# jdidion/atropos

Hardware: AMD Instinct MI355X
Metric: reads/s (whole node) 150 bp SE adapter-align (higher is better)
Workload: dtype int32

## Files before the change

atropos_amd/csrc/filter_core.hpp:

```cpp
#ifndef ATR_FILTER_CORE_HPP
#define ATR_FILTER_CORE_HPP

#include "locate_core.hpp"

namespace atr {

constexpr int FILTER_MAX_M = 64;
constexpr int FILTER_CERT_T = 3;
constexpr int FILTER_CERT_TW = 6;
constexpr int FILTER_BINS = 256;

struct FilterParams {
    uint64_t peq[16];
    int rows;
    int and_mode;
    uint32_t tail;
    int32_t thr_row[FILTER_MAX_M + 1];
    uint32_t cert[FILTER_CERT_T + 1];
    uint64_t cert_sub;
    uint64_t rowsel[4];
    uint32_t tailx[3];
    uint64_t cert64[FILTER_CERT_TW + 1];
};

// ... 106 lines not shown
                bool all = true;
                for (int i = 1; i <= m && all; ++i) if (i != x) all = ok(i, i < x ? o : o - 1);
                threat = all;
            }
        if (!threat) cert |= 1ull << (r - 1);
    }
    return cert;
}

inline FilterParams filter_params(const uint64_t *peq64, const uint8_t *codes, int m, int flags, bool and_mode,
                                  const int16_t *thr, int min_overlap, bool planes_path = false) {
    FilterParams fp;
    fp.rows = m; fp.and_mode = and_mode ? 1 : 0; fp.tail = 0u;
    fp.tailx[0] = fp.tailx[1] = fp.tailx[2] = 0u;
    for (int i = 0; i <= FILTER_MAX_M; ++i)
        fp.thr_row[i] = (i >= 1 && i <= m && i >= min_overlap && ((flags & ATR_STOP_WITHIN_SEQ1) || i == m)) ? (int32_t)thr[i] : -1;
    for (int c = 0; c < 16; ++c) fp.peq[c] = peq64[c];
    (void)planes_path;
    if (filter_narrow_applies(m, flags)) {
        fp.rows = FILTER_NARROW_ROWS;
        for (int c = 0; c < 16; ++c) fp.peq[c] = (peq64[c] >> (64 - m)) & 0xFFFFFFFFull;
        for (int t = 0; t < m - FILTER_NARROW_ROWS; ++t) {
            const uint32_t nib = (uint32_t)(codes[FILTER_NARROW_ROWS + t] & 15u) << (4 * (t & 7));
            if (t < 8) fp.tail |= nib; else fp.tailx[(t >> 3) - 1] |= nib;
        }
    }
    filter_overlap_certificates(codes, m, fp.rows, fp.thr_row, and_mode, fp.cert);
    filter_overlap_certificates64(codes, m, planes_path ? fp.rows : 0, fp.thr_row, and_mode, fp.cert64);
    fp.cert_sub = 0ull;
    fp.rowsel[0] = fp.rowsel[1] = fp.rowsel[2] = fp.rowsel[3] = 0ull;
    if (m <= FILTER_MAX_M && (flags & ATR_STOP_WITHIN_SEQ2) && !(flags & ATR_START_WITHIN_SEQ1) && m >= min_overlap && thr[m] >= 1) {
        const int k = (int)thr[m];
        fp.cert_sub = filter_substitution_certificate(codes, m, k, and_mode);
        if (fp.cert_sub)
            for (int i = 0; i < m; ++i) fp.rowsel[codes[i] == 1 ? 0 : codes[i] == 2 ? 1 : codes[i] == 4 ? 2 : 3] |= 1ull << i;
    }
    return fp;
}

constexpr int BAND_W = 16;
#ifndef ATR_BAND_INTERSECT
#define ATR_BAND_INTERSECT 1
#endif
ATR_DEV uint32_t window_word(int j_lo, int j_hi, bool scan, int rows, bool band) {
    return 0x80000000u | (uint32_t)j_lo | ((uint32_t)j_hi << 10) | (scan ? (1u << 20) : 0u) | ((uint32_t)rows << 21) |
           (band ? (1u << 28) : 0u);
}
ATR_DEV bool window_band(uint32_t w) { return ((w >> 28) & 1u) != 0; }
ATR_DEV int window_rows(uint32_t w) { return (int)((w >> 21) & 0x7Fu); }
ATR_DEV int window_lo(uint32_t w) { return (int)(w & 0x3FFu); }
ATR_DEV int window_hi(uint32_t w) { return (int)((w >> 10) & 0x3FFu); }
ATR_DEV bool window_scan(uint32_t w) { return ((w >> 20) & 1u) != 0; }
ATR_DEV bool window_valid(uint32_t w) { return (w >> 31) != 0; }
ATR_DEV uint32_t last_band_word(int dlo, int top, int span, int width, bool rowm) {
    return window_word(dlo, span | (width << 6), true, top, true) | (rowm ? (1u << 29) : 0u);
}
ATR_DEV int last_band_span(uint32_t w) { return window_hi(w) & 63; }
ATR_DEV int last_band_width(uint32_t w) { return window_hi(w) >> 6; }
ATR_DEV bool last_band_rowm(uint32_t w) { return ((w >> 29) & 1u) != 0; }
constexpr int BAND_BINS = 96, ROWS_BIN0 = 192;
ATR_DEV int triangle_rows(int rows, int n, int j, int k) { return rows - (n - j) + k; }
ATR_DEV bool ragged_rows_bins(bool start_within_seq1) { return !start_within_seq1; }
constexpr int TAIL_COLUMNS = 64;

constexpr int LAST_BIN0 = 32;
ATR_DEV int window_bin(uint32_t w, int m, bool by_rows) {
    const int rows = window_rows(w), start = window_lo(w) >> 3;
    if (window_band(w)) {
        if (window_scan(w)) return LAST_BIN0 + 63 - atr_min(rows, 63);
        const int wide = atr_min(7, atr_max(0, (window_hi(w) - window_lo(w) - m) >> 1));
        return (7 - wide) * 4 + atr_min(3, start >> 4);
    }
    if (rows >= m || !by_rows) return 96 + start;
    return ROWS_BIN0 + atr_min(rows, 63);
}

#ifndef ATR_HOST_EMU
__device__ __forceinline__ void fetch_peq8(const uint2 *peq, uint32_t w, uint2 (&e)[8]) {
#pragma unroll
    for (int b = 0; b < 8; ++b) {
        uint32_t off;
        if (b == 0) off = (w << 3) & 0x78u;
        else asm("v_lshrrev_b32 %0, %1, %2\n\tv_and_b32 %0, 0x78, %0" : "=v"(off) : "n"(4 * b - 3), "v"(w));
        e[b] = *(const uint2 *)((const char *)peq + off);
    }
}
#endif

struct FilterState {
    uint32_t pvl, pvh, mvl, mvh;
    int score;
    uint32_t hits;
    uint32_t nz;
    int zfirst;
    int j_first, j_last;
};

ATR_DEV int filter_row_offset(int m, bool wide) { return (wide ? 64 : 32) - m; }
ATR_DEV int filter_row_offset(int m) { return filter_row_offset(m, m > 32); }

ATR_DEV void filter_init(FilterState &F, const Uniform &u, int mf, bool wide) {
    const int off = filter_row_offset(mf, wide);
    const uint32_t low = off >= 32 ? 0u : ~0u << (off & 31);
    if (wide) { F.pvl = u.sr ? 0u : low; F.pvh = u.sr ? 0u : (off > 32 ? ~0u << (off & 31) : ~0u); }
    else { F.pvl = u.sr ? 0u : low; F.pvh = 0u; }
    F.mvl = F.mvh = 0u;
    F.score = (u.sr ? 0 : mf) - (u.k + 1);
    F.hits = F.nz = 0u;
    F.zfirst = 0;
    F.j_first = F.j_last = 0;
}
ATR_DEV void filter_init(FilterState &F, const Uniform &u, int mf) { filter_init(F, u, mf, mf > 32); }

template <bool WIDE>
ATR_DEV void filter_shift_out2(uint32_t &phl, uint32_t &phh, uint32_t &mhl, uint32_t &mhh, int &score, uint32_t &hits,
                               uint32_t &nz, uint32_t kreg) {
#ifdef ATR_HOST_EMU
    hits = (hits << 1) | ((uint32_t)score >> 31);
    nz = (nz << 1) | (uint32_t)(((uint64_t)(uint32_t)score + (uint64_t)kreg) >> 32);
    const uint32_t pout = WIDE ? phh >> 31 : phl >> 31, mout = WIDE ? mhh >> 31 : mhl >> 31;
    if (WIDE) { phh = (phh << 1) | (phl >> 31); mhh = (mhh << 1) | (mhl >> 31); }
    phl <<= 1; mhl <<= 1;
    score += (int)pout - (int)mout;
#else
    uint64_t c0, c2, c3;
    uint32_t t1, t2;
// ... 123 lines not shown
        const int hoff = off > 32 ? off - 32 : 0, hrows = mf - low_rows;
        const uint32_t q = scan(F.pvh >> hoff, F.mvh >> hoff, low_rows + 1, hrows);
        if (q != 0u) largest = low_rows + hrows - atr_ctz(q);
    }
    if (WIDE) {
        const uint64_t rows = (largest >= 64 ? ~0ull : ((1ull << largest) - 1ull)) << off;
        const uint64_t pv = ((uint64_t)F.pvh << 32) | F.pvl, mv = ((uint64_t)F.mvh << 32) | F.mvl;
        cost_of_largest = atr_popc64(pv & rows) - atr_popc64(mv & rows);
    } else {
        const uint32_t rows = (largest >= 32 ? ~0u : ((1u << largest) - 1u)) << off;
        cost_of_largest = atr_popc64((uint64_t)(F.pvl & rows)) - atr_popc64((uint64_t)(F.mvl & rows));
    }
    d_mf = d;
    row_exact = largest;
    if (tail_rule != 1)
        for (int i = mf + 1; i <= u.m; ++i)
            if ((tail_rule == 2 ? d + (i - mf) : d - (i - mf)) <= fp.thr_row[i]) { largest = i; exact = false; }
    return largest;
}

ATR_DEV uint32_t read_dword(const uint32_t *q, int nchunks, int z8);
template <class P, class DW>
ATR_DEV bool filter_tail_cmp(const P &fp, int T, int jp, DW dw) {
    const uint32_t sh = 4u * (uint32_t)(jp & 7);
    bool ok = true;
    uint32_t lo = dw(jp >> 3);
#pragma unroll
    for (int q = 0; q < FILTER_NARROW_TAIL_EXT / 8; ++q) {
        if (8 * q >= T) break;
        const uint32_t hi = dw((jp >> 3) + q + 1);
        const uint32_t w = sh ? ((lo >> sh) | (hi << (32u - sh))) : lo;
        lo = hi;
        const uint32_t tw = q == 0 ? fp.tail : fp.tailx[q >= 1 ? q - 1 : 0];
        const uint32_t x = fp.and_mode ? (w & tw) : (w ^ tw);
        const int left = T - 8 * q;
        const uint32_t ones = left >= 8 ? 0x11111111u : (0x11111111u & ((1u << (4 * left)) - 1u));
        const uint32_t nz = (x | (x >> 1) | (x >> 2) | (x >> 3)) & ones;
        ok = ok && (fp.and_mode ? nz == ones : nz == 0u);
    }
    return ok;
}
template <class P>
ATR_DEV bool filter_tail_matches(const P &fp, int T, const uint32_t *q, int nchunks, int jp) {
    return filter_tail_cmp(fp, T, jp, [&](int z) { return read_dword(q, nchunks, z); });
}

ATR_DEV uint64_t filter_cert64(const FilterParams &fp, int t) { return fp.cert64[t]; }
template <class P> ATR_DEV uint64_t filter_cert64(const P &, int) { return 0ull; }

struct FilterNoDiag { ATR_DEV_MEMBER uint64_t operator()(int) const { return ~0ull; } };

template <bool WIDE, class P, class TM, class DG = FilterNoDiag>
ATR_DEV uint32_t filter_decide_tm(const FilterState &F, const Uniform &u, const P &fp, TM tm, int n, uint32_t rec[4],
                                  int s = 0, bool have_last = true, DG dg = DG(), int pa_dlo = 0, int pa_dhi = -1) {
    const int mf = fp.rows, T = u.m - mf;
    rec[0] = 0xFFFF0000u; rec[1] = 0; rec[2] = 0; rec[3] = 0;
    if (F.zfirst != 0 && u.m >= u.min_overlap) {
        const int j = F.zfirst + T;
        if (T == 0 || (j <= n && tm(j - T))) {
            rec[0] = (uint32_t)u.m << 16;
            rec[1] = (uint32_t)(j - u.m) | ((uint32_t)j << 16);
            rec[2] = (uint32_t)u.m;
            return 0;
        }
    }
    int cost_l = 0, d_mf = 0, row_e = 0;
    bool exact_l = true;
    const int tail_rule = T == 0 ? 0 : (F.j_first == 0 || F.j_last < n - T - u.k) ? 1 : F.j_first == n ? 2 : 0;
    const int row_l = have_last ? filter_last_column<WIDE>(F, u, fp, cost_l, exact_l, tail_rule, d_mf, row_e) : 0;
    const bool lastcol = row_l != 0;
    const bool rowm = F.j_first != 0 && u.m >= u.min_overlap && !(tail_rule == 2 && d_mf + T > u.k);
    if (!lastcol && !rowm) return 0;
    if (!rowm && !u.sr && exact_l && cost_l == 0) {
        rec[0] = (uint32_t)row_l << 16;
        rec[1] = (uint32_t)(n - row_l) | ((uint32_t)n << 16);
        rec[2] = (uint32_t)row_l;
        return 0;
    }
    if (!WIDE && !rowm && !u.sr && exact_l && u.indel == 1 && cost_l >= 1 && cost_l <= FILTER_CERT_T && row_l > cost_l) {
        const int i = row_l - cost_l, off = filter_row_offset(mf, false);
        const uint32_t seg = ((1u << cost_l) - 1u) << (off + i);
        if ((F.pvl & seg) == seg && ((fp.cert[cost_l] >> i) & 1u) != 0u && n - i >= s) {
            rec[0] = (uint32_t)i << 16;
            rec[1] = (uint32_t)(n - i) | ((uint32_t)n << 16);
            rec[2] = (uint32_t)i;
            return 0;
        }
    }
    if (WIDE && !rowm && !u.sr && exact_l && u.indel == 1 && cost_l >= 1 && cost_l <= FILTER_CERT_TW && row_l > cost_l) {
        const int i = row_l - cost_l, off = filter_row_offset(mf, true);
        const uint64_t seg = ((1ull << cost_l) - 1ull) << (off + i), pv = ((uint64_t)F.pvh << 32) | F.pvl;
        if ((pv & seg) == seg && ((filter_cert64(fp, cost_l) >> i) & 1ull) != 0ull && n - i >= s) {
            rec[0] = (uint32_t)i << 16;
            rec[1] = (uint32_t)(n - i) | ((uint32_t)n << 16);
            rec[2] = (uint32_t)i;
            return 0;
        }
    }
    if (!rowm && !u.sr && exact_l && u.indel == 1) {
        const int kk = atr_min(u.k, (int)fp.thr_row[row_l]), dlo = n - row_l - kk;
        if (dlo >= s && cost_l + 2 * kk <= BAND_W - 1) return last_band_word(dlo, row_l, atr_min(cost_l, row_l - 1), cost_l + 2 * kk, false);
    }
    if (rowm && lastcol && !u.sr && u.indel == 1 && row_e != 0) {
        const int top = exact_l ? row_l : u.m, r0 = atr_max(1, row_e - cost_l);
        const int dlo = atr_min(F.j_first - mf - u.k, n - top - u.k), dhi = atr_max(F.j_last - mf + u.k, n - r0 + u.k);
        if (dlo >= s && dhi - dlo <= BAND_W - 1) return last_band_word(dlo, top, top - r0, dhi - dlo, true);
    }
    int j_lo = 0x7fffffff;
    if (rowm) j_lo = F.j_first - mf - u.k;
    if (lastcol) j_lo = atr_min(j_lo, n - row_l - ((u.indel == 1 && exact_l) ? cost_l : u.k));
    j_lo = atr_max(s, j_lo);
    bool band = rowm && !lastcol && (F.j_first - mf - u.k >= s) &&
                (F.j_last - F.j_first + 2 * u.k <= BAND_W - 1);
    int band_hi = F.j_last + T;
    const bool pa = rowm && !lastcol && !u.sr && pa_dhi >= pa_dlo && pa_dlo > s;
    if (!band && pa && pa_dhi - pa_dlo <= BAND_W - 1) {
        band = true;
        j_lo = pa_dlo;
        band_hi = pa_dhi + u.m - u.k;
    } else if (band && !u.sr && u.indel == 1 && fp.cert_sub != 0ull && ((F.j_first + F.j_last) & 1) == 0 &&
        F.j_last - F.j_first <= 2 * u.k) {
        const int xc = (F.j_first + F.j_last) >> 1, d = xc - mf, j = d + u.m;
        if (d >= s && j <= n) {
            const uint64_t mm = dg(d);
            if (mm != 0ull && (mm & (mm - 1ull)) == 0ull && (mm & fp.cert_sub) != 0ull) {
                rec[0] = (uint32_t)u.m << 16;
                rec[1] = (uint32_t)d | ((uint32_t)j << 16);
                rec[2] = (uint32_t)(u.m - 1) | (1u << 16);
                return 0;
            }
        }
    }
    if (ATR_BAND_INTERSECT && band && pa) {
        const int lo = atr_max(pa_dlo, F.j_first - mf - u.k), hi = atr_min(pa_dhi + u.m - u.k, F.j_last + T);
        if (hi - (u.m - u.k) >= lo) { j_lo = lo; band_hi = hi; }
    }
    const int j_hi = lastcol ? n : band ? band_hi : atr_min(n, F.j_last + (T ? T + u.k : 0));
    return window_word(j_lo, j_hi, lastcol, rowm ? u.m : row_l, band);
}

template <bool WIDE, class P>
ATR_DEV uint32_t filter_decide(const FilterState &F, const Uniform &u, const P &fp, const uint32_t *q,
                               int nchunks, int n, uint32_t rec[4], int s = 0) {
    const int T = u.m - fp.rows;
    return filter_decide_tm<WIDE>(F, u, fp, [&](int jp) { return filter_tail_matches(fp, T, q, nchunks, jp); }, n, rec, s);
}

struct BandParams {
    uint32_t rrep[FILTER_MAX_M];
    int and_mode, noindel;
};

constexpr int BAND_STREAM = (FILTER_MAX_M + BAND_W + 7) / 8 + 1;

ATR_DEV uint32_t read_dword(const uint32_t *q, int nchunks, int z8) {
    if (z8 < 0 || z8 >= nchunks * 4) return 0u;
    return q[(size_t)(z8 >> 2) * 256 + (z8 & 3)];
}

ATR_DEV int band_stream_dwords(int m) { return atr_min(BAND_STREAM, 3 + (m >> 3)); }
ATR_DEV void band_stage(const uint32_t *q, int nchunks, int dlo, uint32_t *ns, int nss, int ndw = BAND_STREAM) {
    const int z0 = dlo >> 3;
    const uint32_t sh = 4u * (uint32_t)(dlo & 7);
    uint32_t raw[BAND_STREAM + 1];
#pragma unroll
    for (int k = 0; k <= BAND_STREAM; ++k) raw[k] = k <= ndw ? read_dword(q, nchunks, z0 + k) : 0u;
#pragma unroll
    for (int k = 0; k < BAND_STREAM; ++k)
        if (k < ndw) ns[(size_t)k * nss] = sh ? ((raw[k] >> sh) | (raw[k + 1] << (32u - sh))) : raw[k];
}

ATR_DEV uint32_t nibble_any(uint32_t v) {
    const uint32_t t = v | (v << 1);
    return t | (t << 2);
}

template <bool AND_MODE, int ND, bool PREFIX = false, class RR>
ATR_DEV void band_rows(const Uniform &u, RR rrep_of, const uint32_t *ns, int nss, uint32_t (&band)[BAND_W]) {
    const uint32_t inf = ((uint32_t)INIT_COST_CAP << CSH) | ORG_BIAS;
    uint32_t qw0 = ns[0], qw1 = ns[(size_t)nss];
    uint32_t feed = ns[(size_t)2 * nss];
    for (int i = 1; i <= u.m; ++i) {
        const uint32_t rrep = rrep_of(i);
        uint32_t m0 = nibble_any(AND_MODE ? (qw0 & rrep) : (qw0 ^ rrep));
        uint32_t m1 = ND > 8 ? nibble_any(AND_MODE ? (qw1 & rrep) : (qw1 ^ rrep)) : 0u;
        if (AND_MODE) { m0 = ~m0; m1 = ~m1; }
        uint32_t left = inf;
        if (PREFIX && i <= u.k) {
            const uint32_t col0 = ORG_BIAS | ((uint32_t)atr_min(i * u.indel, INIT_COST_CAP) << CSH);
#pragma unroll
// ... 215 lines not shown
```

atropos_amd/csrc/locate_core.hpp:

```cpp
#ifndef ATR_LOCATE_CORE_HPP
#define ATR_LOCATE_CORE_HPP

#include <stdint.h>
#include "atropos_hip.h"

#ifdef ATR_HOST_EMU
#define ATR_DEV static inline
#ifndef ATR_DEV_MEMBER
#define ATR_DEV_MEMBER inline
#endif
static inline int atr_min(int a, int b) { return a < b ? a : b; }
static inline int atr_max(int a, int b) { return a > b ? a : b; }
static inline uint32_t atr_minu(uint32_t a, uint32_t b) { return a < b ? a : b; }
static inline uint32_t atr_mad24(uint32_t a, uint32_t b, uint32_t c) { return a * b + c; }
static inline uint32_t atr_bfe1(uint32_t w, int i) { return (w >> i) & 1u; }
static inline int atr_clz(uint32_t w) { return __builtin_clz(w); }
static inline int atr_ctz(uint32_t w) { return __builtin_ctz(w); }
static inline int atr_popc64(uint64_t w) { return __builtin_popcountll(w); }
#else
#define ATR_DEV __device__ __forceinline__
#ifndef ATR_DEV_MEMBER
#define ATR_DEV_MEMBER __device__ __forceinline__
#endif
#define atr_min min
// ... 174 lines not shown
    return u;
}

template <int MT, bool NOINDEL, bool XREP>
ATR_DEV void lane_init(LaneState<MT> &L, const Uniform &u, int n, const uint32_t *s_init, const int16_t *thr) {
    L.n = n;
    L.max_n = u.sq ? n : atr_min(n, u.m + u.k);
    L.min_n = XREP ? 0 : atr_max(0, n - u.m - u.k);
    L.scan = (L.max_n == n);
    if (XREP) {
#pragma unroll
        for (int i = 0; i <= MT; ++i) L.col[i] = s_init[i];
    } else {
#pragma unroll
        for (int i = 0; i <= MT; ++i) L.col[i] = init_word(i - u.p0, L.min_n, u.sr, u.sq, u.indel);
    }
    L.best.key = COST_FIELD_MAX - (u.m + n);
    L.best.word = (uint32_t)(u.m + n) << CSH;
    L.best.ref_stop = u.m; L.best.query_stop = n; L.best.matches = 0;
    if (L.scan && n == 0)
        scan_last_column<MT, XREP>(L.best, L.col, u.p0, u.first_p, n, u.min_overlap, thr, NOINDEL ? 0 : u.indel, u.klimit);
}

ATR_DEV uint32_t window_init_word(int i, int j_lo, int indel) {
    const int cost = i < 0 ? INIT_COST_CAP : atr_min(i * indel, INIT_COST_CAP);
    return ((uint32_t)cost << CSH) | (uint32_t)(j_lo + (int)ORG_BIAS);
}

template <int MT, bool NOINDEL>
ATR_DEV void lane_init_window(LaneState<MT> &L, const Uniform &u, int n, int j_start, int j_hi, bool scan,
                              const uint32_t *s_init, const int16_t *thr) {
    L.n = n; L.min_n = j_start; L.max_n = j_hi; L.scan = scan;
    if (j_start == 0) {
#pragma unroll
        for (int i = 0; i <= MT; ++i) L.col[i] = s_init[i];
    } else {
#pragma unroll
        for (int i = 0; i <= MT; ++i) L.col[i] = window_init_word(i - u.p0, j_start, u.indel);
    }
    L.best.key = COST_FIELD_MAX - (u.m + n);
    L.best.word = (uint32_t)(u.m + n) << CSH;
    L.best.ref_stop = u.m; L.best.query_stop = n; L.best.matches = 0;
    if (scan && j_hi <= j_start)
        scan_last_column<MT, true>(L.best, L.col, u.p0, u.first_p, n, u.min_overlap, thr, NOINDEL ? 0 : u.indel, u.klimit);
}

template <int MT>
ATR_DEV void lane_restart_window(LaneState<MT> &L, const Uniform &u, int j_start) {
#pragma unroll
    for (int i = 0; i <= MT; ++i) L.col[i] = window_init_word(i - u.p0, j_start, u.indel);
    L.best.key = COST_FIELD_MAX - (u.m + L.n);
    L.best.word = (uint32_t)(u.m + L.n) << CSH;
    L.best.ref_stop = u.m; L.best.query_stop = L.n; L.best.matches = 0;
}

template <int MT, bool NOINDEL, bool XREP, bool WIN = false>
ATR_DEV void lane_step(LaneState<MT> &L, const Uniform &u, int j, const uint32_t (&nm)[(MT + 31) / 32],
                       const int16_t *thr, int plimit = MT, int obase = 0) {
    const int indel = NOINDEL ? 0 : u.indel;
    const uint32_t row0 = u.sq ? (ORG_BIAS + (uint32_t)(j - obase))
                               : (ORG_BIAS | ((uint32_t)atr_min(j * u.indel, INIT_COST_CAP) << CSH));
    const uint32_t wm = WIN ? column_step_limited<MT, NOINDEL, XREP>(L.col, nm, u.p0, row0, u.insw, u.delw, plimit)
                            : column_step<MT, NOINDEL, XREP>(L.col, nm, u.p0, row0, u.insw, u.delw);
    if (WIN) {
        if (plimit == MT && wm < u.klimit && j <= L.max_n)
            consider<XREP>(L.best, wm, u.m, j, u.min_overlap, thr, indel);
    } else if (XREP) {
        if (wm < u.klimit && j <= L.max_n) consider<XREP>(L.best, wm, u.m, j, u.min_overlap, thr, indel, obase);
    } else if (j == L.min_n && L.max_n > L.min_n) {
        int mn = L.min_n;
#ifndef ATR_HOST_EMU
        asm volatile("" : "+v"(mn));
#endif
#pragma unroll
        for (int i = 0; i <= MT; ++i) L.col[i] = init_word(i - u.p0, mn, u.sr, u.sq, u.indel) - (uint32_t)obase;
    }
    if (L.scan && j == L.max_n && L.max_n > L.min_n)
        scan_last_column<MT, XREP>(L.best, L.col, u.p0, u.first_p, L.n, u.min_overlap, thr, indel, u.klimit, WIN ? plimit : MT, obase);
}

constexpr int LONG_BASE_STEP = 256, LONG_MAX_SPAN = 384;
ATR_DEV int long_base(int j) { return j > 2 * LONG_BASE_STEP ? (((j - 1) / LONG_BASE_STEP) - 1) * LONG_BASE_STEP : 0; }
template <int MT>
ATR_DEV void lane_rebase(LaneState<MT> &L) {
#pragma unroll
    for (int i = 0; i <= MT; ++i) {
        const uint32_t w = L.col[i];
        L.col[i] = (w & ORG_MASK) >= (uint32_t)LONG_BASE_STEP ? w - (uint32_t)LONG_BASE_STEP : (w & ~ORG_MASK);
    }
}

template <int MT>
ATR_DEV void lane_result(const LaneState<MT> &L, const Uniform &u, uint32_t rec[4], int obase = 0) {
    const int cost = (int)(L.best.word >> CSH);
    int refstart = 0, querystart = 0, refstop = -1, querystop = 0, matches = 0, errors = 0;
    if (L.best.key != COST_FIELD_MAX - (u.m + L.n) && cost != u.m + L.n) {
        const int origin = (int)(L.best.word & ORG_MASK) - (int)ORG_BIAS + obase;
        if (origin >= 0) querystart = origin; else refstart = -origin;
        refstop = L.best.ref_stop; querystop = L.best.query_stop;
        matches = L.best.matches; errors = cost;
    }
    rec[0] = (uint32_t)(refstart & 0xFFFF) | ((uint32_t)(refstop & 0xFFFF) << 16);
    rec[1] = (uint32_t)(querystart & 0xFFFF) | ((uint32_t)(querystop & 0xFFFF) << 16);
    rec[2] = (uint32_t)(matches & 0xFFFF) | ((uint32_t)(errors & 0xFFFF) << 16);
    rec[3] = 0;
}
// ... 45 lines not shown
```

atropos_amd/csrc/locate_fast.hpp:

```cpp
#ifndef ATR_LOCATE_FAST_HPP
#define ATR_LOCATE_FAST_HPP

#include <algorithm>
#include "locate_kernel.hpp"
#include "filter_core.hpp"
#include "linked_core.hpp"
#include "piece_core.hpp"
#include "fast_work.hpp"

namespace atr {
inline const FilterParams &aligner_filter_params(const atr_aligner *a) {
    struct Slot { unsigned long long uid = 0; FilterParams fp; };
    static thread_local Slot slots[4];
    static thread_local unsigned turn = 0;
    if (a->uid != 0)
        for (Slot &s : slots) if (s.uid == a->uid) return s.fp;
    Slot &s = slots[turn++ & 3u];
    s.fp = filter_params(a->peq, a->codes, a->p.m, a->flags, a->wildcard_ref || a->wildcard_query, a->p.thr, a->p.min_overlap);
    s.uid = a->uid;
    return s.fp;
}
inline const FilterParams &aligner_piece_filter_params(const atr_aligner *a) {
    struct Slot { unsigned long long uid = 0; FilterParams fp; };
    static thread_local Slot slots[4];
// ... 257 lines not shown
    __syncthreads();
    const int lane = threadIdx.x & 63;
    const long long tile = (long long)blockIdx.x * 4 + __builtin_amdgcn_readfirstlane((int)(threadIdx.x >> 6));
    if (tile * 64 >= nreads) return;
    const long long r = tile * 64 + lane;
    const bool live = r < nreads;
    const int n = live ? (lens ? lens[r] : max_len) : 0;
    const uint32_t *q = (const uint32_t *)(packed + (size_t)tile * nchunks * 64 + lane);
    uint32_t *ns = &s_stream[__builtin_amdgcn_readfirstlane((int)(threadIdx.x >> 6))][0][lane];
    band_stage(q, nchunks, -u.k, ns, 64, band_stream_dwords(u.m));
    uint32_t rec[4];
    band_locate_prefix<AND_MODE>(u, bp.rrep, bp.noindel != 0, ns, 64, n, s_thr, rec);
    if (live) out[r] = make_uint4(rec[0], rec[1], rec[2], rec[3]);
}
#endif

template <bool LINKED>
__device__ __forceinline__ const LocateParams &window_params(const LocateParams &p_arg, const LinkedArgs &la, int ad) {
    if constexpr (LINKED) return la.multi_p[ad];
    else return p_arg;
}

template <int MT, bool NOINDEL, bool LINKED, bool PLANES = false>
__global__ __launch_bounds__(256) void window_kernel(const LocateParams p_arg, const uint4 *__restrict__ packed,
                                                     const int32_t *__restrict__ lens, long long nreads,
                                                     int nchunks, int max_len, uint4 *__restrict__ out, FastWork wk,
                                                     const LinkedArgs la) {
    __shared__ int16_t s_thr[ATR_MAX_REF_LEN + 2];
    __shared__ uint32_t s_init[ATR_MAX_REF_LEN + 1];
    __shared__ __attribute__((aligned(16))) uint32_t s_nm[16][4];
    __shared__ uint32_t s_spread_flat[PLANES ? 1024 : 1];
    uint32_t (*s_spread)[256] = (uint32_t (*)[256])s_spread_flat;
    const int ad = LINKED ? la.a0 + (int)blockIdx.y : 0;
    const LocateParams &p = window_params<LINKED>(p_arg, la, ad);
    const Uniform u = make_uniform(p, MT);
    if (threadIdx.x < 64) s_nm[threadIdx.x >> 2][threadIdx.x & 3] = p.nmask[threadIdx.x >> 2][threadIdx.x & 3];
    for (int i = threadIdx.x; i <= MT + 1; i += 256) {
        if (i <= u.m + 1) s_thr[i] = p.thr[i];
        if (i <= MT) s_init[i] = init_word(i - u.p0, 0, u.sr, u.sq, u.indel);
    }
    if constexpr (PLANES) piece_spread_fill(s_spread);
    __syncthreads();
    const int bin0 = LINKED ? ad * FILTER_BINS : 0;
    const long long first = (long long)wk.binbase[bin0 + BAND_BINS], total = (long long)wk.binbase[bin0 + FILTER_BINS];
    const int lane = threadIdx.x & 63;
    const int lpw = dp_lanes_per_wave(total - first, (long long)gridDim.x * 4, wk.lpw);
    const long long nwaves = (total - first + lpw - 1) / lpw;
    for (long long wv = (long long)blockIdx.x * 4 + __builtin_amdgcn_readfirstlane((int)(threadIdx.x >> 6)); wv < nwaves;
         wv += (long long)gridDim.x * 4) {
        const long long slot = first + wv * lpw + lane;
        const bool live = lane < lpw && slot < total;
        const uint2 task = live ? wk.order[slot] : make_uint2(0u, 0u);
        const long long r = (long long)task.x;
        const uint32_t ww = task.y;
        const int n = live ? (lens ? lens[r] : max_len) : 0;
        const int j_lo = window_lo(ww), j_hi = live ? window_hi(ww) : 0;
        const bool has_window = live && j_hi > j_lo;
        const int jlo = wave_min_i32(live ? j_lo : 0x7fffffff);
        const int jhi = wave_max_i32(has_window ? j_hi : 0);
        const int rows_w = wave_max_i32(live ? window_rows(ww) : 0);
        const int plimit = u.p0 + rows_w;
        const bool head = !(u.sr && jlo == 0);
        const bool tri = __builtin_amdgcn_readfirstlane((int)(first + wv * lpw >= (long long)wk.binbase[bin0 + ROWS_BIN0])) != 0 &&
                         head && lens == nullptr;
        const int s_lane = (LINKED && live) ? (int)(la.front[r].y >> 16) : 0;
        const int s_top = LINKED ? wave_max_i32(s_lane) : 0;

        LaneState<MT> L;
        const uint4 *tp = packed + ((size_t)(r >> 6) * nchunks) * 64 + (r & 63);

        const bool rows_wave = __builtin_amdgcn_readfirstlane((int)(first + wv * lpw >= (long long)wk.binbase[bin0 + ROWS_BIN0])) != 0;
        if (!LINKED && lens != nullptr && rows_wave && !u.sr) {
            const int shift = live ? max_len - n : 0;
            const int v0 = wave_min_i32(live ? j_lo + shift : 0x7fffffff);
            if (max_len - v0 <= TAIL_COLUMNS && v0 < max_len) {
                const int s_top_t = wave_max_i32(shift);
                lane_init_window<MT, NOINDEL>(L, u, max_len, v0, live ? max_len : 0, live && window_scan(ww), s_init, s_thr);
                uint32_t tb[TAIL_COLUMNS / 8];
                {
                    const int dlo = n - TAIL_COLUMNS;
                    const int z0 = dlo >> 3;
                    const uint32_t sh = 4u * (uint32_t)(dlo & 7);
                    uint32_t raw[TAIL_COLUMNS / 8 + 1];
#pragma unroll
                    for (int t = 0; t <= TAIL_COLUMNS / 8; ++t) {
                        if constexpr (PLANES) raw[t] = live ? read_dword_planes((const uint32_t *)tp, nchunks, z0 + t, s_spread) : 0u;
                        else raw[t] = live ? read_dword((const uint32_t *)tp, nchunks, z0 + t) : 0u;
                    }
#pragma unroll
                    for (int t = 0; t < TAIL_COLUMNS / 8; ++t) tb[t] = sh ? ((raw[t] >> sh) | (raw[t + 1] << (32u - sh))) : raw[t];
                }
                int j = max_len - TAIL_COLUMNS;
#pragma unroll 1
                for (int d = 0; d < TAIL_COLUMNS / 8; ++d) {
                    uint32_t w = tb[0];
#pragma unroll
                    for (int t = 0; t + 1 < TAIL_COLUMNS / 8; ++t) tb[t] = tb[t + 1];
#pragma unroll 1
                    for (int b = 0; b < 8; ++b) {
                        ++j;
                        const uint32_t q = w & 15u;
                        w >>= 4;
                        if (j <= v0) continue;
                        uint32_t nm[(MT + 31) / 32];
                        load_mask(nm, s_nm, q);
                        int pl = min(plimit, u.p0 + (j - v0) + u.k);
                        pl = min(pl, u.p0 + triangle_rows(rows_w, max_len, j, u.k));
                        lane_step<MT, NOINDEL, true, true>(L, u, j, nm, s_thr, pl);
// ... 87 lines not shown
```

atropos_amd/csrc/piece_filter.hpp:

```cpp
#ifndef ATR_PIECE_FILTER_HPP
#define ATR_PIECE_FILTER_HPP

#include "fast_work.hpp"
#include "pack_fast.hpp"

namespace atr {

#ifndef ATR_PIECE_PREFETCH_EARLY
#define ATR_PIECE_PREFETCH_EARLY 1
#endif
#ifndef ATR_PIECE_STASH
#define ATR_PIECE_STASH 1
#endif
#ifndef ATR_PIECE_WAVES
#if defined(ATR_SPEC) && defined(ATR_SPEC_ASCII)
#define ATR_PIECE_WAVES(NW) 2
#elif defined(ATR_SPEC)
#define ATR_PIECE_WAVES(NW) ((NW) <= 6 ? 4 : 3)
#else
#define ATR_PIECE_WAVES(NW) ((NW) <= 6 ? 4 : (NW) <= 8 ? 3 : 2)
#endif
#endif

constexpr int PIECE_QF = 2;
template <bool B> struct PieceBool { static constexpr bool value = B; };

__device__ __forceinline__ int lane_rank(uint64_t mask) {
    return (int)__builtin_amdgcn_mbcnt_hi((uint32_t)(mask >> 32), __builtin_amdgcn_mbcnt_lo((uint32_t)mask, 0u));
}

__device__ __forceinline__ void piece_emit(bool active, long long r, uint32_t ww, const uint32_t (&rec)[4], int m, uint4 *out,
                                           uint2 *list, uint4 *ldata, const uint32_t *nibs, int j0, uint32_t *s_lcur, uint32_t *s_hist,
                                           int nd = 8) {
    const bool open = active && window_valid(ww);
    if (active && !open) out[r] = make_uint4(rec[0], rec[1], rec[2], rec[3]);
    const uint64_t om = __ballot(open);
    if (om != 0ull) {
        uint32_t base = 0u;
        if ((threadIdx.x & 63) == 0) base = atomicAdd(s_lcur, (uint32_t)__popcll(om));
        base = __builtin_amdgcn_readfirstlane(base);
        const int lane = threadIdx.x & 63;
        const int off = window_lo(ww) - j0;
        const bool dense = nibs != nullptr && off >= 0 && off < 64 && band_stream_dwords(m) <= 8;
        if (open) {
            const uint32_t slot = base + (uint32_t)lane_rank(om);
            list[slot] = make_uint2((uint32_t)r, dense ? ww : (ww | PIECE_NODENSE));
            atomicAdd(&s_hist[window_bin(ww, m, true)], 1u);
            if (dense) {
                const int z = off >> 3;
                const uint32_t sh = 4u * (uint32_t)(off & 7);
                uint32_t raw[9], d[8];
#pragma unroll
                for (int k = 0; k < 9; ++k) raw[k] = z + k < nd ? nibs[(z + k) * 64 + lane] : 0u;
#pragma unroll
                for (int k = 0; k < 8; ++k) d[k] = sh ? ((raw[k] >> sh) | (raw[k + 1] << (32u - sh))) : raw[k];
                ldata[2 * (size_t)slot] = make_uint4(d[0], d[1], d[2], d[3]);
                ldata[2 * (size_t)slot + 1] = make_uint4(d[4], d[5], d[6], d[7]);
            }
        }
    }
}

template <int NW, bool RAGGED, int WW = 2>
__device__ __forceinline__ void piece_filter_body(const LocateParams &p, const FilterParams &fp_arg, const PieceParams &pp_arg,
                                                  const uint4 *__restrict__ planes, const int32_t *__restrict__ lens,
                                                  long long nreads, int max_len, uint4 *__restrict__ out, FastWork wk,
                                                  const uint8_t *__restrict__ ascii = nullptr, const uint8_t *tab = nullptr) {
#ifdef ATR_SPEC
    if (!RAGGED) max_len = spec::N;
#endif
#ifdef ATR_SPEC_ASCII
    static_assert(NW <= 8, "the fused ASCII entry keeps pass B's window in the LDS stash");
    constexpr int STRIDE = ATR_SPEC_STRIDE;
    constexpr int NPC = (15 + 64 * STRIDE + 1023) / 1024;
    constexpr int STAGE_BYTES = (64 * STRIDE + PACK_STAGE_SLACK + 15) & ~15;
    __shared__ __attribute__((aligned(16))) uint8_t s_stage[4][STAGE_BYTES];
// ... 92 lines not shown
            nb[d] = 0u;
            if (d >= dw0 - 1) nb[d] = piece_nibbles(s_spread, wp[0][d >> 2], wp[1][d >> 2], wp[2][d >> 2], wp[3][d >> 2], d & 3);
            nibs[d * 64 + lane] = nb[d];
        }
        const auto sweep_decide = [&](auto wc) __attribute__((always_inline)) {
        constexpr bool WD = decltype(wc)::value;
        FilterState F;
        filter_init(F, u, mf, WD);
        int vstart = 0;
        if (u.sr) {
            const bool zero0 = j_e - W <= 0;
            Uniform uf = u;
            uf.sr = false;
            FilterState G;
            filter_init(G, uf, mf, WD);
            if (!zero0) { F.pvl = G.pvl; F.pvh = G.pvh; F.score = G.score; }
            vstart = zero0 ? PW - j_e : 0;
        }
        uint2 ea[8], eb[8];
#pragma unroll
        for (int d = 0; d < ND; ++d) {
            if (d < dw0) continue;
            uint2 (&e)[8] = (d & 1) ? eb : ea;
            if (d == dw0) fetch_peq8(s_peq, nb[d], e);
            if (d + 1 < ND) fetch_peq8(s_peq, nb[d + 1], (d & 1) ? ea : eb);
            if (u.sr) {
#pragma unroll
                for (int b = 0; b < 8; ++b) if (8 * d + b < vstart) { e[b].x = ~0u; e[b].y = ~0u; }
            }
#pragma unroll
            for (int b = 0; b < 8; ++b) filter_step<WD>(F, e[b].x, e[b].y, kreg);
            if ((d & 3) == 3 && d + 1 < ND) filter_fold(F, j_e - PW + 8 * (d + 1), mf, kreg);
        }
        filter_fold(F, j_e, mf, kreg);
        uint32_t rec[4];
        const auto tm = [&](int jp) {
            const int rp = max(0, jp - (j_e - PW));
            return filter_tail_cmp(fp, T, rp, [&](int z) { return z < ND ? nibs[z * 64 + lane] : 0u; });
        };
        const auto dg = [&](int d) -> uint64_t {
            if constexpr (WW != 2 || WD) return ~0ull;
            const int o = d - (j_e - PW);
            if (o < 0 || o + u.m > PW) return ~0ull;
            uint64_t eq = 0ull;
#pragma unroll
            for (int c = 0; c < 4; ++c) {
                uint32_t lo = wp[c][0], hi = wp[c][1];
#pragma unroll
                for (int q = 0; q < 4; ++q) if (q != c && !fp.and_mode) { lo &= ~wp[q][0]; hi &= ~wp[q][1]; }
                eq |= ((((uint64_t)hi << 32) | lo) >> o) & fp.rowsel[c];
            }
            return ~eq & (u.m >= 64 ? ~0ull : (1ull << u.m) - 1ull);
        };
        const uint32_t ww = filter_decide_tm<WD>(F, u, fp, tm, nr, rec, 0, j_e == nr, dg, j_e - need, j_e < nr ? j_e - u.m : -0x10000);
        piece_emit(act, r, ww, rec, u.m, out, list, ldata, nibs, j_e - PW, &s_lcur, s_hist, ND);
        };
        if (mf > 32) {
            if constexpr (WIDE_OK) sweep_decide(PieceBool<true>{});
        } else {
            sweep_decide(PieceBool<false>{});
        }
    };

    int qn = 0;

#ifdef ATR_SPEC_ASCII
    uint4 ax[NPC];
    const auto ascii_edge = [&](long long tile) {
        const uint8_t *src = ascii + tile * 64 * STRIDE;
        const uint8_t *al = src - ((uintptr_t)src & 15);
        const long long need = (long long)((uintptr_t)src & 15) + (nreads - tile * 64 < 64 ? nreads - tile * 64 : 64) * STRIDE;
        return al < ascii || al + ((need + 15) & ~15ll) > buf_end;
    };
    const auto ascii_request = [&](long long tile) {
        if (ascii_edge(tile)) return;
        const uint8_t *src = ascii + tile * 64 * STRIDE;
        const uint8_t *al = src - ((uintptr_t)src & 15);
        const long long need = (long long)((uintptr_t)src & 15) + (nreads - tile * 64 < 64 ? nreads - tile * 64 : 64) * STRIDE;
#pragma unroll
        for (int u = 0; u < NPC; ++u) {
            const long long o = (long long)u * 1024 + (long long)lane * 16;
            ax[u] = o < need ? *(const uint4 *)(al + o) : make_uint4(0u, 0u, 0u, 0u);
        }
    };
    if (t0 + wave < t1) ascii_request(t0 + wave);
#else
    uint4 nx[NW];
    if (t0 + wave < t1) {
        const uint4 *tp = planes + (size_t)(t0 + wave) * NW * 64;
#pragma unroll
        for (int w = 0; w < NW; ++w) nx[w] = tp[w * 64 + lane];
    }
#endif
    for (long long tile = t0 + wave; tile < t1; tile += 4) {
        const long long r = tile * 64 + lane;
        const bool live = r < nreads;
        uint32_t pl[NW][4];
#ifdef ATR_SPEC_ASCII
        {
            uint8_t *stage = s_stage[wave];
            uint32_t mis;
            if (ascii_edge(tile)) {
                mis = pack_stage_tile(stage, ascii, STRIDE, nreads, tile, lane);
            } else {
                const uint8_t *src = ascii + tile * 64 * STRIDE;
                mis = (uint32_t)((uintptr_t)src & 15);
                const long long need = (long long)mis + (nreads - tile * 64 < 64 ? nreads - tile * 64 : 64) * STRIDE;
// ... 126 lines not shown
                }
            };
            if (narrow && rank < room) put(qn + rank);
            if (cnt >= room) {
                __builtin_amdgcn_fence(__ATOMIC_RELEASE, "wavefront");
                pass_b(64);
                __builtin_amdgcn_fence(__ATOMIC_RELEASE, "wavefront");
                if (narrow && rank >= room) put(rank - room);
                qn = cnt - room;
            } else {
                qn += cnt;
            }
        }
    }
    __builtin_amdgcn_fence(__ATOMIC_RELEASE, "wavefront");
    if (qn > 0) pass_b(qn);
    __threadfence_block();
    __syncthreads();
    {
        const long long total = (long long)s_wcnt;
        for (long long base = (long long)wave * 64; base < total; base += 256) {
            const bool act = base + lane < total;
            const long long r = act ? (long long)wlist[base + lane] : t0 * 64;
            const uint4 *bp = planes + ((size_t)(r >> 6) * NW) * 64 + (r & 63);
            const uint4 *tp = bp;
            const size_t tstride = 64;
            const int nl = RAGGED ? (act ? min(max(lens[r], 0), max_len) : 0) : max_len;
            const int nhi = RAGGED ? wave_max_i32(nl) : max_len;
            const auto full_sweep = [&](auto wc) __attribute__((always_inline)) {
            constexpr bool WD = decltype(wc)::value;
            FilterState F;
            filter_init(F, u, mf, WD);
            int j = 0;
#pragma clang loop unroll(disable)
            for (int c = 0; c < NW; ++c) {
                if (j >= nhi) break;
                const uint4 v = tp[(size_t)c * tstride];
#pragma clang loop unroll(disable)
                for (int d = 0; d < 4; ++d) {
                    if (j >= nhi) break;
                    uint2 e[8];
                    fetch_peq8(s_peq, piece_nibbles(s_spread, v.x, v.y, v.z, v.w, d), e);
#pragma unroll
                    for (int b = 0; b < 8; ++b)
                        if (j + b < nl) filter_step<WD>(F, e[b].x, e[b].y, kreg);
                    j += 8;
                }
                filter_fold(F, min(j, nl), mf, kreg);
            }
            uint32_t rec[4];
            const auto tm = [&](int jp) {
                return filter_tail_cmp(fp, T, jp, [&](int z) { return read_dword_planes((const uint32_t *)bp, NW, z, s_spread); });
            };
            const uint32_t ww = filter_decide_tm<WD>(F, u, fp, tm, nl, rec, 0, true);
            piece_emit(act, r, ww, rec, u.m, out, list, ldata, nullptr, 0, &s_lcur, s_hist);
            };
            if (mf > 32) {
                if constexpr (WIDE_OK) full_sweep(PieceBool<true>{});
            } else {
                full_sweep(PieceBool<false>{});
            }
        }
    }
    __syncthreads();
    fused_hist_flush(wk, s_hist);
    if (threadIdx.x == 0) wk.lcount[blockIdx.x] = s_lcur;
}

}
#endif
```

atropos_amd/csrc/tail_filter.hpp:

```cpp
#ifndef ATR_TAIL_FILTER_HPP
#define ATR_TAIL_FILTER_HPP

#ifdef ATR_HOST_EMU
#include "filter_core.hpp"
#else
#include "fast_work.hpp"
#endif

namespace atr {

#ifndef ATR_TAIL_ROWS_UNROLL
#define ATR_TAIL_ROWS_UNROLL 8
#endif
#ifndef ATR_TAIL_WINDOW_UNROLL
#define ATR_TAIL_WINDOW_UNROLL 2
#endif
constexpr int TAIL_ROWS_UNROLL = ATR_TAIL_ROWS_UNROLL;
static_assert(TAIL_ROWS_UNROLL >= 8 && TAIL_ROWS_UNROLL % 8 == 0, "the feed position is a compile-time place of the body");

template <bool AND_MODE, int ND>
ATR_DEV void tail_band_row(const Uniform &u, uint32_t rrep, uint32_t qw0, uint32_t qw1, uint32_t (&band)[BAND_W]) {
    const uint32_t inf = ((uint32_t)INIT_COST_CAP << CSH) | ORG_BIAS;
    uint32_t m0 = nibble_any(AND_MODE ? (qw0 & rrep) : (qw0 ^ rrep));
    uint32_t m1 = ND > 8 ? nibble_any(AND_MODE ? (qw1 & rrep) : (qw1 ^ rrep)) : 0u;
// ... 195 lines not shown
        const bool dense = live && (ww & PIECE_NODENSE) == 0u;
        if (dense) {
            ns[0] = a.x; ns[64] = a.y; ns[128] = a.z; ns[192] = a.w;
            ns[256] = b.x; ns[320] = b.y; ns[384] = b.z; ns[448] = b.w;
        }
        if (wave_max_i32(live && !dense ? 1 : 0) != 0) {
            const uint32_t *q = (const uint32_t *)(packed + ((size_t)(r >> 6) * nchunks) * 64 + (r & 63));
            if (live && !dense) band_stage_planes(q, nchunks, window_lo(ww), ns, 64, S.spread, band_stream_dwords(M));
        }
        uint32_t rec[4] = {0xFFFF0000u, 0u, 0u, 0u};
        if (any_rowm) tail_band_locate<tspec::AND_MODE, M>(u, tspec::RREP, tspec::NOINDEL, ns, 64, n, ww, smax, S.thr, rec);
        if (any_last) {
            const int smax_l = min(BAND_W - 1, wave_max_i32(last ? last_band_width(ww) : 0));
            const int rows_max = wave_max_i32(last ? (last_band_rowm(ww) ? u.m : window_rows(ww)) : 0);
            const int cap_lo = wave_min_i32(last ? window_rows(ww) - last_band_span(ww) : 0x7fffffff);
            uint32_t rec_l[4];
            tail_band_locate_last<tspec::AND_MODE, M>(u, tspec::RREP, tspec::NOINDEL, ns, 64, n, ww, last, smax_l, min(rows_max, M), cap_lo, S.thr, rec_l);
            if (last) { rec[0] = rec_l[0]; rec[1] = rec_l[1]; rec[2] = rec_l[2]; rec[3] = rec_l[3]; }
        }
        if (live) out[r] = make_uint4(rec[0], rec[1], rec[2], rec[3]);
        task = task1; di = di1; a = a1; b = b1; n = n1;
        task1 = task2; di1 = di2;
    }
}

template <int W>
__device__ __forceinline__ void tail_load_mask(uint32_t (&nm)[W], const uint32_t (*s_nm)[4], uint32_t q) {
#pragma unroll
    for (int w = 0; w < W; ++w) nm[w] = s_nm[q][w];
}

__device__ __forceinline__ void tail_window_blocks(TailShared &S, int block, int nblocks, const uint4 *__restrict__ packed,
                                                   const int32_t *__restrict__ lens, int nchunks, int max_len,
                                                   uint4 *__restrict__ out, const FastWork &wk) {
    constexpr int MT = tspec::MT;
    constexpr bool NOINDEL = tspec::NOINDEL;
    const Uniform u = tail_uniform();
    const int16_t *s_thr = S.thr;
    const uint32_t *s_init = S.init;
    const uint32_t (*s_nm)[4] = S.nm;
    const uint32_t (*s_spread)[256] = S.spread;
    const long long first = (long long)wk.binbase[BAND_BINS], total = (long long)wk.binbase[FILTER_BINS];
    if (total <= first) return;
    const int lane = threadIdx.x & 63;
    const int lpw = tail_lanes_per_wave(total - first, (long long)nblocks * 4, wk.lpw);
    const long long nwaves = (total - first + lpw - 1) / lpw;
    __builtin_amdgcn_s_setprio(3);
    for (long long wv = (long long)block * 4 + __builtin_amdgcn_readfirstlane((int)(threadIdx.x >> 6)); wv < nwaves;
         wv += (long long)nblocks * 4) {
        const long long slot = first + wv * lpw + lane;
        const bool live = lane < lpw && slot < total;
        const uint2 task = live ? wk.order[slot] : make_uint2(0u, 0u);
        const long long r = (long long)task.x;
        const uint32_t ww = task.y;
        const int n = live ? (lens ? lens[r] : max_len) : 0;
        const int j_lo = window_lo(ww), j_hi = live ? window_hi(ww) : 0;
        const bool has_window = live && j_hi > j_lo;
        const int jlo = wave_min_i32(live ? j_lo : 0x7fffffff);
        const int jhi = wave_max_i32(has_window ? j_hi : 0);
        const int rows_w = wave_max_i32(live ? window_rows(ww) : 0);
        const int plimit = u.p0 + rows_w;
        const bool head = !(u.sr && jlo == 0);
        const bool rows_wave = __builtin_amdgcn_readfirstlane((int)(first + wv * lpw >= (long long)wk.binbase[ROWS_BIN0])) != 0;
        const bool tri = rows_wave && head && lens == nullptr;

        LaneState<MT> L;
        const uint4 *tp = packed + ((size_t)(r >> 6) * nchunks) * 64 + (r & 63);

        if (lens != nullptr && rows_wave && !u.sr) {
            const int shift = live ? max_len - n : 0;
            const int v0 = wave_min_i32(live ? j_lo + shift : 0x7fffffff);
            if (max_len - v0 <= TAIL_COLUMNS && v0 < max_len) {
                const int s_top_t = wave_max_i32(shift);
                lane_init_window<MT, NOINDEL>(L, u, max_len, v0, live ? max_len : 0, live && window_scan(ww), s_init, s_thr);
                uint32_t tb[TAIL_COLUMNS / 8];
                {
                    const int dlo = n - TAIL_COLUMNS;
                    const int z0 = dlo >> 3;
                    const uint32_t sh = 4u * (uint32_t)(dlo & 7);
                    uint32_t raw[TAIL_COLUMNS / 8 + 1];
#pragma unroll
                    for (int t = 0; t <= TAIL_COLUMNS / 8; ++t)
                        raw[t] = live ? read_dword_planes((const uint32_t *)tp, nchunks, z0 + t, s_spread) : 0u;
#pragma unroll
                    for (int t = 0; t < TAIL_COLUMNS / 8; ++t) tb[t] = sh ? ((raw[t] >> sh) | (raw[t + 1] << (32u - sh))) : raw[t];
                }
                int j = max_len - TAIL_COLUMNS;
#pragma unroll 1
                for (int d = 0; d < TAIL_COLUMNS / 8; ++d) {
                    uint32_t w = tb[0];
#pragma unroll
                    for (int t = 0; t + 1 < TAIL_COLUMNS / 8; ++t) tb[t] = tb[t + 1];
#pragma unroll 1
                    for (int b = 0; b < 8; ++b) {
                        ++j;
                        const uint32_t q = w & 15u;
                        w >>= 4;
                        if (j <= v0) continue;
                        uint32_t nm[(MT + 31) / 32];
                        tail_load_mask(nm, s_nm, q);
                        int pl = min(plimit, u.p0 + (j - v0) + u.k);
                        pl = min(pl, u.p0 + triangle_rows(rows_w, max_len, j, u.k));
                        lane_step<MT, NOINDEL, true, true>(L, u, j, nm, s_thr, pl);
                        if (j <= s_top_t && shift == j) lane_restart_window<MT>(L, u, j);
                    }
                }
                if (live) {
                    uint32_t rec[4];
                    lane_result<MT>(L, u, rec);
                    if ((rec[0] >> 16) != 0xFFFFu) rec[1] -= (uint32_t)shift * 0x00010001u;
                    out[r] = make_uint4(rec[0], rec[1], rec[2], rec[3]);
                }
                continue;
            }
        }
        lane_init_window<MT, NOINDEL>(L, u, n, jlo, j_hi, live && window_scan(ww), s_init, s_thr);
        if (jhi > jlo) {
            const int c0 = jlo >> 5, c1 = (jhi + 31) >> 5;
            uint4 nxt = tp[(size_t)c0 * 64];
            for (int c = c0; c < c1; ++c) {
                uint4 cur = nxt;
                if (c + 1 < c1) nxt = tp[(size_t)(c + 1) * 64];
                cur = make_uint4(piece_nibbles(s_spread, cur.x, cur.y, cur.z, cur.w, 0), piece_nibbles(s_spread, cur.x, cur.y, cur.z, cur.w, 1),
                                 piece_nibbles(s_spread, cur.x, cur.y, cur.z, cur.w, 2), piece_nibbles(s_spread, cur.x, cur.y, cur.z, cur.w, 3));
                int j = c * 32;
#pragma unroll 1
                for (int d = 0; d < 4; ++d) {
                    uint32_t w = cur.x;
                    cur.x = cur.y; cur.y = cur.z; cur.z = cur.w;
#pragma unroll ATR_TAIL_WINDOW_UNROLL
                    for (int b = 0; b < 8; ++b) {
                        ++j;
                        const uint32_t q = w & 15u;
                        w >>= 4;
                        if (j <= jlo || j > jhi) continue;
                        uint32_t nm[(MT + 31) / 32];
                        tail_load_mask(nm, s_nm, q);
                        int pl = head ? min(plimit, u.p0 + (j - jlo) + u.k) : plimit;
                        if (tri) pl = min(pl, u.p0 + triangle_rows(rows_w, max_len, j, u.k));
                        lane_step<MT, NOINDEL, true, true>(L, u, j, nm, s_thr, pl);
                    }
                }
            }
        }
        if (live) {
            uint32_t rec[4];
            lane_result<MT>(L, u, rec);
            out[r] = make_uint4(rec[0], rec[1], rec[2], rec[3]);
        }
    }
}

__device__ __forceinline__ void tail_body(const uint4 *__restrict__ packed, const int32_t *__restrict__ lens, int nchunks,
                                          int max_len, uint4 *__restrict__ out, const FastWork &wk, int win_blocks) {
    __shared__ TailShared S;
    for (int i = threadIdx.x; i <= tspec::MT + 1; i += 256) {
        if (i <= tspec::M + 1) S.thr[i] = tspec::THR[i];
        if (i <= tspec::MT) S.init[i] = init_word(i - (tspec::MT - tspec::M), 0, (tspec::FLAGS & ATR_START_WITHIN_SEQ1) != 0,
                                                  (tspec::FLAGS & ATR_START_WITHIN_SEQ2) != 0, tspec::INDEL);
    }
    if (threadIdx.x < 64) S.nm[threadIdx.x >> 2][threadIdx.x & 3] = tspec::NMASK[threadIdx.x >> 2][threadIdx.x & 3];
    piece_spread_fill(S.spread);
    __syncthreads();
    const int block = (int)blockIdx.x, nblocks = (int)gridDim.x;
    if (block < win_blocks) tail_window_blocks(S, block, win_blocks, packed, lens, nchunks, max_len, out, wk);
    else tail_band_blocks(S, block - win_blocks, nblocks - win_blocks, packed, lens, nchunks, max_len, out, wk);
}
#endif

}
#endif
```

Measured before the change: 24.81 billion.

## Split row-limited windows into head and tail segments to skip middle columns

```diff
diff --git a/atropos_amd/csrc/filter_core.hpp b/atropos_amd/csrc/filter_core.hpp
--- a/atropos_amd/csrc/filter_core.hpp
+++ b/atropos_amd/csrc/filter_core.hpp
@@ -182,6 +182,14 @@
 ATR_DEV int window_hi(uint32_t w) { return (int)((w >> 10) & 0x3FFu); }
 ATR_DEV bool window_scan(uint32_t w) { return ((w >> 20) & 1u) != 0; }
 ATR_DEV bool window_valid(uint32_t w) { return (w >> 31) != 0; }
+#ifndef ATR_WINDOW_SPLIT
+#define ATR_WINDOW_SPLIT 1
+#endif
+ATR_DEV bool window_split(uint32_t w) { return ((w >> 28) & 3u) == 2u; }
+ATR_DEV uint32_t window_unsplit(uint32_t w, int n, int m) {
+    if (!window_split(w)) return w;
+    return (w & 0xC00003FFu) | ((uint32_t)n << 10) | (1u << 20) | ((uint32_t)m << 21);
+}
 ATR_DEV uint32_t last_band_word(int dlo, int top, int span, int width, bool rowm) {
     return window_word(dlo, span | (width << 6), true, top, true) | (rowm ? (1u << 29) : 0u);
 }
@@ -201,7 +209,7 @@
         const int wide = atr_min(7, atr_max(0, (window_hi(w) - window_lo(w) - m) >> 1));
         return (7 - wide) * 4 + atr_min(3, start >> 4);
     }
-    if (rows >= m || !by_rows) return 96 + start;
+    if (rows >= m || !by_rows || window_split(w)) return 96 + start;
     return ROWS_BIN0 + atr_min(rows, 63);
 }
 
@@ -431,7 +439,8 @@
 
 template <bool WIDE, class P, class TM, class DG = FilterNoDiag>
 ATR_DEV uint32_t filter_decide_tm(const FilterState &F, const Uniform &u, const P &fp, TM tm, int n, uint32_t rec[4],
-                                  int s = 0, bool have_last = true, DG dg = DG(), int pa_dlo = 0, int pa_dhi = -1) {
+                                  int s = 0, bool have_last = true, DG dg = DG(), int pa_dlo = 0, int pa_dhi = -1,
+                                  bool split_ok = false) {
     const int mf = fp.rows, T = u.m - mf;
     rec[0] = 0xFFFF0000u; rec[1] = 0; rec[2] = 0; rec[3] = 0;
     if (F.zfirst != 0 && u.m >= u.min_overlap) {
@@ -515,6 +524,11 @@
         if (hi - (u.m - u.k) >= lo) { j_lo = lo; band_hi = hi; }
     }
     const int j_hi = lastcol ? n : band ? band_hi : atr_min(n, F.j_last + (T ? T + u.k : 0));
+    if (ATR_WINDOW_SPLIT && split_ok && rowm && lastcol && exact_l && row_l < u.m && u.sq && u.eq && !u.sr && s == 0) {
+        const int j_mid = atr_min(n, F.j_last + (T ? T + u.k : 0));
+        if (j_mid > j_lo && j_mid < n - row_l - u.k)
+            return window_word(j_lo, j_mid, true, row_l, false) | (1u << 29);
+    }
     return window_word(j_lo, j_hi, lastcol, rowm ? u.m : row_l, band);
 }
 
diff --git a/atropos_amd/csrc/locate_core.hpp b/atropos_amd/csrc/locate_core.hpp
--- a/atropos_amd/csrc/locate_core.hpp
+++ b/atropos_amd/csrc/locate_core.hpp
@@ -250,6 +250,13 @@
     L.best.key = COST_FIELD_MAX - (u.m + L.n);
     L.best.word = (uint32_t)(u.m + L.n) << CSH;
     L.best.ref_stop = u.m; L.best.query_stop = L.n; L.best.matches = 0;
+}
+
+template <int MT>
+ATR_DEV void lane_next_segment(LaneState<MT> &L, const Uniform &u, int j_start, int j_hi, bool scan) {
+#pragma unroll
+    for (int i = 0; i <= MT; ++i) L.col[i] = window_init_word(i - u.p0, j_start, u.indel);
+    L.min_n = j_start; L.max_n = j_hi; L.scan = scan;
 }
 
 template <int MT, bool NOINDEL, bool XREP, bool WIN = false>
diff --git a/atropos_amd/csrc/locate_fast.hpp b/atropos_amd/csrc/locate_fast.hpp
--- a/atropos_amd/csrc/locate_fast.hpp
+++ b/atropos_amd/csrc/locate_fast.hpp
@@ -333,8 +333,8 @@
         const bool live = lane < lpw && slot < total;
         const uint2 task = live ? wk.order[slot] : make_uint2(0u, 0u);
         const long long r = (long long)task.x;
-        const uint32_t ww = task.y;
         const int n = live ? (lens ? lens[r] : max_len) : 0;
+        const uint32_t ww = window_unsplit(task.y, n, u.m);
         const int j_lo = window_lo(ww), j_hi = live ? window_hi(ww) : 0;
         const bool has_window = live && j_hi > j_lo;
         const int jlo = wave_min_i32(live ? j_lo : 0x7fffffff);
diff --git a/atropos_amd/csrc/piece_filter.hpp b/atropos_amd/csrc/piece_filter.hpp
--- a/atropos_amd/csrc/piece_filter.hpp
+++ b/atropos_amd/csrc/piece_filter.hpp
@@ -22,6 +22,11 @@
 #endif
 #endif
 
+#ifdef ATR_SPEC
+constexpr bool PIECE_SPLIT = ATR_WINDOW_SPLIT != 0;
+#else
+constexpr bool PIECE_SPLIT = false;
+#endif
 constexpr int PIECE_QF = 2;
 template <bool B> struct PieceBool { static constexpr bool value = B; };
 
@@ -220,7 +225,7 @@
             }
             return ~eq & (u.m >= 64 ? ~0ull : (1ull << u.m) - 1ull);
         };
-        const uint32_t ww = filter_decide_tm<WD>(F, u, fp, tm, nr, rec, 0, j_e == nr, dg, j_e - need, j_e < nr ? j_e - u.m : -0x10000);
+        const uint32_t ww = filter_decide_tm<WD>(F, u, fp, tm, nr, rec, 0, j_e == nr, dg, j_e - need, j_e < nr ? j_e - u.m : -0x10000, PIECE_SPLIT && !RAGGED);
         piece_emit(act, r, ww, rec, u.m, out, list, ldata, nibs, j_e - PW, &s_lcur, s_hist, ND);
         };
         if (mf > 32) {
@@ -453,7 +458,7 @@
             const auto tm = [&](int jp) {
                 return filter_tail_cmp(fp, T, jp, [&](int z) { return read_dword_planes((const uint32_t *)bp, NW, z, s_spread); });
             };
-            const uint32_t ww = filter_decide_tm<WD>(F, u, fp, tm, nl, rec, 0, true);
+            const uint32_t ww = filter_decide_tm<WD>(F, u, fp, tm, nl, rec, 0, true, FilterNoDiag(), 0, -1, PIECE_SPLIT && !RAGGED);
             piece_emit(act, r, ww, rec, u.m, out, list, ldata, nullptr, 0, &s_lcur, s_hist);
             };
             if (mf > 32) {
diff --git a/atropos_amd/csrc/tail_filter.hpp b/atropos_amd/csrc/tail_filter.hpp
--- a/atropos_amd/csrc/tail_filter.hpp
+++ b/atropos_amd/csrc/tail_filter.hpp
@@ -271,13 +271,16 @@
         const bool live = lane < lpw && slot < total;
         const uint2 task = live ? wk.order[slot] : make_uint2(0u, 0u);
         const long long r = (long long)task.x;
-        const uint32_t ww = task.y;
         const int n = live ? (lens ? lens[r] : max_len) : 0;
+        const bool sp = ATR_WINDOW_SPLIT != 0 && lens == nullptr && live && window_split(task.y);
+        const int rows2_w = wave_max_i32(sp ? window_rows(task.y) : 0), s2_w = max_len - rows2_w - u.k;
+        const bool two = rows2_w > 0 && wave_max_i32(live && !sp ? 1 : 0) == 0 && wave_max_i32(sp ? window_hi(task.y) : 0) < s2_w;
+        const uint32_t ww = two ? task.y : window_unsplit(task.y, n, u.m);
         const int j_lo = window_lo(ww), j_hi = live ? window_hi(ww) : 0;
         const bool has_window = live && j_hi > j_lo;
         const int jlo = wave_min_i32(live ? j_lo : 0x7fffffff);
         const int jhi = wave_max_i32(has_window ? j_hi : 0);
-        const int rows_w = wave_max_i32(live ? window_rows(ww) : 0);
+        const int rows_w = two ? u.m : wave_max_i32(live ? window_rows(ww) : 0);
         const int plimit = u.p0 + rows_w;
         const bool head = !(u.sr && jlo == 0);
         const bool rows_wave = __builtin_amdgcn_readfirstlane((int)(first + wv * lpw >= (long long)wk.binbase[ROWS_BIN0])) != 0;
@@ -333,9 +336,17 @@
                 continue;
             }
         }
-        lane_init_window<MT, NOINDEL>(L, u, n, jlo, j_hi, live && window_scan(ww), s_init, s_thr);
-        if (jhi > jlo) {
-            const int c0 = jlo >> 5, c1 = (jhi + 31) >> 5;
+        lane_init_window<MT, NOINDEL>(L, u, n, jlo, j_hi, live && !two && window_scan(ww), s_init, s_thr);
+        int seg_lo = jlo, seg_hi = jhi, seg_pl = plimit, seg_rows = rows_w;
+        bool seg_tri = tri;
+#pragma unroll 1
+        for (int seg = 0; seg < (two ? 2 : 1); ++seg) {
+        if (seg == 1) {
+            lane_next_segment<MT>(L, u, s2_w, n, live);
+            seg_lo = s2_w; seg_hi = max_len; seg_pl = u.p0 + rows2_w; seg_rows = rows2_w; seg_tri = true;
+        }
+        if (seg_hi > seg_lo) {
+            const int c0 = seg_lo >> 5, c1 = (seg_hi + 31) >> 5;
             uint4 nxt = tp[(size_t)c0 * 64];
             for (int c = c0; c < c1; ++c) {
                 uint4 cur = nxt;
@@ -352,15 +363,16 @@
                         ++j;
                         const uint32_t q = w & 15u;
                         w >>= 4;
-                        if (j <= jlo || j > jhi) continue;
+                        if (j <= seg_lo || j > seg_hi) continue;
                         uint32_t nm[(MT + 31) / 32];
                         tail_load_mask(nm, s_nm, q);
-                        int pl = head ? min(plimit, u.p0 + (j - jlo) + u.k) : plimit;
-                        if (tri) pl = min(pl, u.p0 + triangle_rows(rows_w, max_len, j, u.k));
+                        int pl = head ? min(seg_pl, u.p0 + (j - seg_lo) + u.k) : seg_pl;
+                        if (seg_tri) pl = min(pl, u.p0 + triangle_rows(seg_rows, max_len, j, u.k));
                         lane_step<MT, NOINDEL, true, true>(L, u, j, nm, s_thr, pl);
                     }
                 }
             }
+        }
         }
         if (live) {
             uint32_t rec[4];
@@ -382,10 +394,17 @@
     piece_spread_fill(S.spread);
     __syncthreads();
     const int block = (int)blockIdx.x, nblocks = (int)gridDim.x;
-    if (block < win_blocks) tail_window_blocks(S, block, win_blocks, packed, lens, nchunks, max_len, out, wk);
-    else tail_band_blocks(S, block - win_blocks, nblocks - win_blocks, packed, lens, nchunks, max_len, out, wk);
-}
-#endif
-
-}
-#endif
+    if (block < win_blocks) {
+#ifndef ATR_X_TAIL_NOWINDOW
+        tail_window_blocks(S, block, win_blocks, packed, lens, nchunks, max_len, out, wk);
+#endif
+    } else {
+#ifndef ATR_X_TAIL_NOBAND
+        tail_band_blocks(S, block - win_blocks, nblocks - win_blocks, packed, lens, nchunks, max_len, out, wk);
+#endif
+    }
+}
+#endif
+
+}
+#endif
```

After: 24.66 billion. No clear change (-0.6%).
